# ZhenghaoFei/visual_odom

Hardware: NVIDIA H100
Metric: stereo frames/sec at 1241x376, 2000 feats; LK kernel HBM GB/s vs roofline (higher is better)
Workload: dtype u8/i32 fixed point + f32 (LK), f64 (pose)

## Files before the change

### visual_odom_b200/csrc/batch.cu

```cuda
#include "ctx.h"
#include <string.h>
#include <algorithm>

__global__ void k_pack_counts(vo_unit_result_dev* res, const int* n_pts, const int* n_det, const int* n3, const int* n5,
                              int n_units, int detect)
{
    const int u = blockIdx.x * blockDim.x + threadIdx.x;
    if (u >= n_units) return;
    res[u].n_features = n_pts[u];
    res[u].n_detected = detect ? n_det[u] : 0;
    res[u].n_tracked = n3[u];
    res[u].n_valid = n5[u];
}

#define VO_OUT_BYTES_PER_SLOT (4 * sizeof(float2) + sizeof(int) + sizeof(float3) + sizeof(int))
__global__ void k_pack_outputs(uint8_t* __restrict__ out, size_t stride, int per, const float2* __restrict__ valid4, size_t cs,
                               const int* __restrict__ idx5, const float3* __restrict__ X, const int* __restrict__ inliers,
                               const int* __restrict__ n5, const vo_unit_result_dev* __restrict__ res, int cap)
{
    const int u = blockIdx.x;
    const int nv = min(n5[u], per), ni = min(res[u].n_inliers, per);
    float2* o4 = reinterpret_cast<float2*>(out + (size_t)u * stride);
    int* ok = reinterpret_cast<int*>(o4 + 4 * (size_t)per);
    float* oX = reinterpret_cast<float*>(ok + per);
// ... 159 lines not shown
    char who[64];
    snprintf(who, sizeof(who), "vo_batch_submit_device: unit %d", u);
    const vo_dimage* imgs[4] = {&U.l0, &U.r0, &U.l1, &U.r1};
    static const char* names[4] = {"l0", "r0", "l1", "r1"};
    for (int k = 0; k < 4; k++) {
        const int rc = vo_check_dimage(ctx, who, names[k], imgs[k], ctx->w);
        if (rc) return rc;
    }
    return VO_OK;
}

template <typename Unit>
static int validate_units(vo_ctx* ctx, const Unit* units, int n_units, size_t pitch, bool* detect_out, int* max_pts_out = nullptr)
{
    if (!ctx || !units) return VO_E_INVALID;
    if (n_units <= 0 || n_units > ctx->batch_units) { vo_set_error(ctx, "n_units=%d outside the configured batch (%d)", n_units, ctx->batch_units); return VO_E_INVALID; }
    const bool detect = (units[0].pts == nullptr);
    int max_pts = 0;
    for (int u = 0; u < n_units; u++) {
        const Unit& U = units[u];
        int rc = check_images(ctx, U, u, pitch);
        if (rc) return rc;
        if ((U.pts == nullptr) != detect) { vo_set_error(ctx, "units must all carry features or all request detection"); return VO_E_INVALID; }
        if (U.n_pts < 0 || U.n_pts > ctx->cap) { vo_set_error(ctx, "unit %d: n_pts=%d outside [0,%d]", u, U.n_pts, ctx->cap); return VO_E_CAPACITY; }
        if (U.n_pts > max_pts) max_pts = U.n_pts;
    }
    *detect_out = detect;
    if (max_pts_out) *max_pts_out = max_pts;
    return vo_ensure_pinned(ctx, batch_pinned_bytes(ctx));
}

extern "C" int vo_batch_upload(vo_ctx* ctx, const vo_unit* units, int n_units, size_t pitch)
{
    bool detect;
    int rc = validate_units(ctx, units, n_units, pitch, &detect);
    if (rc) return rc;
    VO_CUDA_CHECK(cudaSetDevice(ctx->device));
    if ((rc = vo_claim_buffers(ctx, "vo_batch_upload", true))) return rc;
    if ((rc = vo_drain_pending(ctx))) return rc;
    VO_CUDA_CHECK(cudaStreamSynchronize(ctx->stream));
    if ((rc = upload_range(ctx, units, 0, n_units, pitch, ctx->stream, detect))) return rc;
    ctx->batch_uploaded = n_units;
    ctx->batch_detect = detect;
    return VO_OK;
}

static int ensure_helpers(vo_ctx* ctx)
{
    if (ctx->lane[0].pre) return VO_OK;
    int lo = 0, hi = 0;
    VO_CUDA_CHECK(cudaDeviceGetStreamPriorityRange(&lo, &hi));
    for (auto& L : ctx->lane) {
        VO_CUDA_CHECK(cudaStreamCreateWithPriority(&L.pre, cudaStreamNonBlocking, hi));
        L.post = L.pre;
        L.lk = L.side;
    }
    return VO_OK;
}

static int run_range_launch(vo_ctx* ctx, const View& v)
{
    int rc;
    View pre = v, lk = v, post = v;
    cudaEvent_t* ev = nullptr;
    for (auto& L : ctx->lane)
        if (L.side && v.s == L.side) {
            if ((rc = ensure_helpers(ctx))) return rc;
            pre.s = L.pre; lk.s = L.lk; post.s = L.post; ev = L.ev;
        }
    auto hand_over = [&](int k, cudaStream_t from, cudaStream_t to) -> int {
        if (from == to) return VO_OK;
        VO_CUDA_CHECK(cudaEventRecord(ev[k], from));
        VO_CUDA_CHECK(cudaStreamWaitEvent(to, ev[k], 0));
        return VO_OK;
    };
    if ((rc = hand_over(0, v.s, pre.s))) return rc;
    if (ctx->batch_detect) {
        if ((rc = vo_run_fast(ctx, pre, 0, false))) return rc;
        if ((rc = vo_run_select(ctx, pre))) return rc;
    }
    if ((rc = vo_run_pyramid(ctx, v.u0 * v.imgs, v.n * v.imgs, pre.s))) return rc;
    if ((rc = hand_over(1, pre.s, lk.s))) return rc;
    const int ip[4] = {0, 1, 3, 2}, in[4] = {1, 3, 2, 0};
    if ((rc = vo_run_lk_ring(ctx, lk, 4, ip, in, false))) return rc;
    if ((rc = hand_over(2, lk.s, post.s))) return rc;
    if ((rc = vo_run_filter(ctx, post, false))) return rc;
    const size_t cs = (size_t)ctx->units * ctx->cap;
    if ((rc = vo_run_triangulate(ctx, post, ctx->d_valid4, ctx->d_valid4 + cs, ctx->d_n5, ctx->d_cal))) return rc;
    if ((rc = vo_run_pnp(ctx, post, ctx->d_valid4 + 2 * cs, ctx->d_n5, ctx->d_cal))) return rc;
    k_pack_counts<<<(v.n + 63) / 64, 64, 0, post.s>>>(ctx->d_results + v.u0, ctx->d_npts + v.u0, ctx->d_ndet + v.u0, ctx->d_n3 + v.u0,
                                                     ctx->d_n5 + v.u0, v.n, ctx->batch_detect ? 1 : 0);
    ctx->launches += 1;
    VO_CUDA_CHECK(cudaGetLastError());
    return hand_over(3, post.s, v.s);
}

static int run_range(vo_ctx* ctx, int u0, int n, cudaStream_t s)
{
    View v{u0, n, s};
    v.max_pts = range_bound(ctx, u0, n);
    bool on_side = false;
    for (const auto& L : ctx->lane) on_side = on_side || (L.side && s == L.side);
    if (on_side) return run_range_launch(ctx, v);
    GraphKey key{};
    key.kind = GraphKey::BATCH_RANGE; key.s = s; key.tma = ctx->lk_use_tma;
    key.u0 = u0; key.n = n; key.max_pts = v.max_pts; key.detect = ctx->batch_detect;
    return vo_run_graph(ctx, key, [&] { return run_range_launch(ctx, v); });
}

extern "C" int vo_batch_run(vo_ctx* ctx)
{
    if (!ctx) return VO_E_INVALID;
    const int units = ctx->batch_uploaded;
    if (units <= 0) { vo_set_error(ctx, "vo_batch_run: nothing uploaded"); return VO_E_INVALID; }
    { int rcc = vo_claim_buffers(ctx, "vo_batch_run"); if (rcc) return rcc; }
    VO_CUDA_CHECK(cudaSetDevice(ctx->device));
    if (units < 2 || ctx->batch_streams < 2) return run_range(ctx, 0, units, ctx->stream);
    int rc = vo_ensure_lanes(ctx);
    if (rc) return rc;
    VO_CUDA_CHECK(cudaEventRecord(ctx->fork_ev, ctx->stream));
    const int half = (units + 1) / 2;
    for (int c = 0; c < 2; c++) {
        const int u0 = c ? half : 0, n = c ? units - half : half;
        cudaStream_t st = ctx->lane[c].side;
        VO_CUDA_CHECK(cudaStreamWaitEvent(st, ctx->fork_ev, 0));
        if ((rc = run_range(ctx, u0, n, st))) return rc;
        VO_CUDA_CHECK(cudaEventRecord(ctx->lane[c].join, st));
        VO_CUDA_CHECK(cudaStreamWaitEvent(ctx->stream, ctx->lane[c].join, 0));
    }
    return VO_OK;
}

extern "C" int vo_batch_download(vo_ctx* ctx, vo_unit_result* results, int n_units)
{
    if (!ctx || !results) return VO_E_INVALID;
    if (n_units <= 0 || n_units > ctx->batch_uploaded) { vo_set_error(ctx, "n_units=%d outside the resident batch (%d)", n_units, ctx->batch_uploaded); return VO_E_INVALID; }
    static_assert(sizeof(vo_unit_result) == sizeof(vo_unit_result_dev), "result record layout");
    VO_CUDA_CHECK(cudaSetDevice(ctx->device));
    VO_CUDA_CHECK(cudaMemcpyAsync(results, ctx->d_results, (size_t)n_units * sizeof(vo_unit_result), cudaMemcpyDeviceToHost, ctx->stream));
    VO_CUDA_CHECK(cudaStreamSynchronize(ctx->stream));
    return VO_OK;
}

extern "C" int vo_frame_batch(vo_ctx* ctx, const vo_unit* units, int n_units, size_t pitch, vo_unit_result* results)
{
    bool detect;
// ... 192 lines not shown
```

### visual_odom_b200/csrc/ctx.cu

```cuda
#include "ctx.h"
#include <string.h>
#include <stdlib.h>

void vo_set_error(vo_ctx* ctx, const char* fmt, ...)
{
    if (!ctx) return;
    va_list ap;
    va_start(ap, fmt);
    vsnprintf(ctx->err, sizeof(ctx->err), fmt, ap);
    va_end(ap);
}

extern "C" void vo_default_params(vo_params* p)
{
    p->fast_threshold = 20;
    p->fast_nonmax = 1;
    p->lk_win = 21;
    p->lk_max_level = 3;
    p->lk_max_iters = 30;
    p->lk_epsilon = 0.01;
    p->lk_min_eig = 0.001;
    p->circ_threshold = 0;
    p->pnp_iterations = 500;
    p->pnp_reproj_error = 0.5f;
    p->pnp_confidence = (double)0.999f;
    p->max_features = 8192;
    p->max_units = 1;
}

extern "C" int vo_create(int device, const vo_params* params, vo_ctx** out)
{
    if (!out) return VO_E_INVALID;
    *out = nullptr;
    vo_ctx* ctx = new vo_ctx();
    if (params) ctx->p = *params; else vo_default_params(&ctx->p);
    ctx->device = device;
    *out = ctx;
    if (ctx->p.fast_threshold < 0 || ctx->p.fast_threshold > 255) {
        vo_set_error(ctx, "fast_threshold=%d outside [0,255]", ctx->p.fast_threshold);
        return VO_E_INVALID;
    }
    if (ctx->p.lk_win != VO_WIN) {
        vo_set_error(ctx, "lk_win=%d unsupported: the LK kernel is built for the reference's 21x21 window", ctx->p.lk_win);
        return VO_E_UNSUPPORTED;
    }
    if (ctx->p.lk_max_level < 0 || ctx->p.lk_max_level >= VO_MAX_LEVELS) {
        vo_set_error(ctx, "lk_max_level=%d outside [0,%d]", ctx->p.lk_max_level, VO_MAX_LEVELS - 1);
        return VO_E_UNSUPPORTED;
    }
    int ndev = 0;
    cudaError_t e = cudaGetDeviceCount(&ndev);
    if (e != cudaSuccess || ndev <= 0) {
        vo_set_error(ctx, "no CUDA device available (%s): this library has no CPU fallback", cudaGetErrorString(e));
        return VO_E_CUDA;
    }
    VO_CUDA_CHECK(cudaSetDevice(device));
    cudaDeviceProp prop;
    VO_CUDA_CHECK(cudaGetDeviceProperties(&prop, device));
    if (prop.major != 9 || prop.minor != 0) {
        vo_set_error(ctx, "device %d is sm_%d%d; this library ships sm_90a code only", device, prop.major, prop.minor);
        return VO_E_UNSUPPORTED;
    }
    ctx->sm_count = prop.multiProcessorCount;
    VO_CUDA_CHECK(cudaStreamCreateWithFlags(&ctx->own_stream, cudaStreamNonBlocking));
    ctx->stream = ctx->own_stream;
    VO_CUDA_CHECK(vo_lk_prepare());
    ctx->cap = ctx->p.max_features;
    VO_CUDA_CHECK(cudaMalloc(&ctx->d_lk_queue, LK_QUEUES * 2 * sizeof(int)));
    VO_CUDA_CHECK(cudaMemset(ctx->d_lk_queue, 0, LK_QUEUES * 2 * sizeof(int)));
    {
        const char* st = getenv("VO_LK_STAGING");
        ctx->lk_use_tma = !(st && strcmp(st, "ldg") == 0);
        const char* sp = getenv("VO_LK_SPAN");
        if (sp) ctx->lk_span = atoi(sp);
    }
    return VO_OK;
}

extern "C" void vo_destroy(vo_ctx* ctx)
{
    if (!ctx) return;
    cudaSetDevice(ctx->device);
    vo_drain_pending(ctx);
    if (ctx->stream) cudaStreamSynchronize(ctx->stream);
    vo_dist_shutdown(ctx);
    vo_partition_destroy(ctx);
    vo_free_state(ctx);
    for (cudaEvent_t e : ctx->ev_pool) cudaEventDestroy(e);
    for (auto& p : ctx->pending) if (p.done) cudaEventDestroy(p.done);
    for (int k = 0; k < 2; k++) {
        if (ctx->seq_front_ev[k]) cudaEventDestroy(ctx->seq_front_ev[k]);
        if (ctx->seq_back_ev[k]) cudaEventDestroy(ctx->seq_back_ev[k]);
    }
    if (ctx->fork_ev) cudaEventDestroy(ctx->fork_ev);
    for (auto& L : ctx->lane) {
        if (L.join) cudaEventDestroy(L.join);
        if (L.side) cudaStreamDestroy(L.side);
        for (cudaEvent_t e : L.ev) if (e) cudaEventDestroy(e);
    }
    if (ctx->h_pinned) cudaFreeHost(ctx->h_pinned);
    if (ctx->d_bgr) cudaFree(ctx->d_bgr);
    if (ctx->d_lk_queue) cudaFree(ctx->d_lk_queue);
    if (ctx->d_ess) cudaFree(ctx->d_ess);
    if (ctx->d_seq_ess) cudaFree(ctx->d_seq_ess);
    for (int k = 0; k < 2; k++) if (ctx->seq_mono_ev[k]) cudaEventDestroy(ctx->seq_mono_ev[k]);
    if (ctx->seq_mono_stream) cudaStreamDestroy(ctx->seq_mono_stream);
    if (ctx->h_out) cudaFreeHost(ctx->h_out);
    if (ctx->own_stream) cudaStreamDestroy(ctx->own_stream);
    delete ctx;
}

extern "C" const char* vo_last_error(const vo_ctx* ctx) { return ctx ? ctx->err : "null context"; }

extern "C" int vo_set_stream(vo_ctx* ctx, void* s)
{
    if (!ctx) return VO_E_INVALID;
    VO_CUDA_CHECK(cudaStreamSynchronize(ctx->stream));
    ctx->stream = s ? (cudaStream_t)s : ctx->own_stream;
    return VO_OK;
}

extern "C" int vo_sync(vo_ctx* ctx)
{
    if (!ctx) return VO_E_INVALID;
    VO_CUDA_CHECK(cudaStreamSynchronize(ctx->stream));
    return VO_OK;
}

extern "C" int vo_set_option(vo_ctx* ctx, const char* key, double value)
{
    if (!ctx || !key) return VO_E_INVALID;
    if (strcmp(key, "batch_streams") == 0) { ctx->batch_streams = value >= 2 ? 2 : 1; return VO_OK; }
    if (strcmp(key, "lk_staging") == 0) { ctx->lk_use_tma = !(value >= 1); return VO_OK; }
    if (strcmp(key, "batch_outputs") == 0) { ctx->batch_outputs = value >= 1; vo_drop_graphs(ctx); return VO_OK; }
    if (strcmp(key, "sm_partition") == 0) {
        if (value < 0) { vo_set_error(ctx, "sm_partition=%g: the number of SMs must not be negative", value); return VO_E_INVALID; }
        ctx->part_auto = false;
        return vo_partition_enable(ctx, (int)value);
    }
    if (strcmp(key, "lk_span") == 0) { ctx->lk_span = (int)value; vo_drop_graphs(ctx); return VO_OK; }
    if (strcmp(key, "graphs") == 0) { ctx->use_graphs = value >= 1; return VO_OK; }
    if (strcmp(key, "mono_rotation") == 0) { ctx->mono_opt = value >= 1; vo_drop_graphs(ctx); return VO_OK; }
    vo_set_error(ctx, "unknown option %s", key);
    return VO_E_INVALID;
}

extern "C" long long vo_kernel_launches(const vo_ctx* ctx) { return ctx ? ctx->launches : 0; }

extern "C" int vo_lk_kernel_time(vo_ctx* ctx, double* ms_total, long long* n, int reset)
{
    if (!ctx) return VO_E_INVALID;
    VO_CUDA_CHECK(cudaStreamSynchronize(ctx->stream));
    for (size_t i = 0; i + 1 < ctx->ev_used; i += 2) {
        float ms = 0.f;
        VO_CUDA_CHECK(cudaEventElapsedTime(&ms, ctx->ev_pool[i], ctx->ev_pool[i + 1]));
        ctx->lk_ms += ms;
        ctx->lk_n++;
    }
    ctx->ev_used = 0;
    if (ms_total) *ms_total = ctx->lk_ms;
    if (n) *n = ctx->lk_n;
    if (reset) { ctx->lk_ms = 0.0; ctx->lk_n = 0; }
    return VO_OK;
}

int vo_ensure_pinned(vo_ctx* ctx, size_t bytes)
{
    if (bytes <= ctx->h_pinned_bytes) return VO_OK;
    if (ctx->h_pinned) { cudaFreeHost(ctx->h_pinned); ctx->h_pinned = nullptr; ctx->h_pinned_bytes = 0; }
    VO_CUDA_CHECK(cudaMallocHost(&ctx->h_pinned, bytes));
    ctx->h_pinned_bytes = bytes;
    return VO_OK;
}

int vo_upload_plane(vo_ctx* ctx, uint8_t* dst, const uint8_t* src, size_t row_bytes, int h, size_t pitch, cudaStream_t st)
{
    if (pitch == row_bytes) VO_CUDA_CHECK(cudaMemcpyAsync(dst, src, row_bytes * h, cudaMemcpyHostToDevice, st));
    else VO_CUDA_CHECK(cudaMemcpy2DAsync(dst, row_bytes, src, pitch, row_bytes, h, cudaMemcpyHostToDevice, st));
    return VO_OK;
}

int vo_refuse_pending_batches(vo_ctx* ctx, const char* who)
{
    for (auto& p : ctx->pending)
        if (p.active) {
            vo_set_error(ctx, "%s: the vo_batch_submit submission of slots [%d, %d) has not been waited for", who, p.u0, p.u0 + p.n);
            return VO_E_INVALID;
        }
    return VO_OK;
}

int vo_claim_buffers(vo_ctx* ctx, const char* who, bool allow_pending_batches)
{
    if (ctx->seq_inflight > 0) {
        vo_set_error(ctx, "%s: %d frame(s) submitted with vo_seq_submit have not been waited for (this call would overwrite their buffers)", who, ctx->seq_inflight);
        return VO_E_INVALID;
    }
    int rc;
    if (!allow_pending_batches && (rc = vo_refuse_pending_batches(ctx, who))) return rc;
    ctx->seq_active = false;
    return VO_OK;
}

typedef CUresult (*PFN_cuDeviceGet)(CUdevice*, int);
typedef CUresult (*PFN_cuDeviceGetDevResource)(CUdevice, CUdevResource*, CUdevResourceType);
typedef CUresult (*PFN_cuDevSmResourceSplitByCount)(CUdevResource*, unsigned int*, const CUdevResource*, CUdevResource*, unsigned int, unsigned int);
typedef CUresult (*PFN_cuDevResourceGenerateDesc)(CUdevResourceDesc*, CUdevResource*, unsigned int);
typedef CUresult (*PFN_cuGreenCtxCreate)(CUgreenCtx*, CUdevResourceDesc, CUdevice, unsigned int);
typedef CUresult (*PFN_cuGreenCtxStreamCreate)(CUstream*, CUgreenCtx, unsigned int, int);
typedef CUresult (*PFN_cuGreenCtxDestroy)(CUgreenCtx);

template <typename F>
static bool drv(const char* name, F* fn)
{
    void* p = nullptr;
    cudaDriverEntryPointQueryResult q;
    if (cudaGetDriverEntryPoint(name, &p, cudaEnableDefault, &q) != cudaSuccess || q != cudaDriverEntryPointSuccess || !p) return false;
    *fn = (F)p;
    return true;
}

void vo_partition_destroy(vo_ctx* ctx)
{
    for (auto& L : ctx->lane) {
        if (L.pre) cudaStreamDestroy(L.pre);
        if (L.post && L.post != L.pre) cudaStreamDestroy(L.post);
        L.pre = L.lk = L.post = nullptr;
    }
    PFN_cuGreenCtxDestroy destroy = nullptr;
    if (drv("cuGreenCtxDestroy", &destroy))
        for (int k = 0; k < 2; k++) if (ctx->part_gctx[k]) destroy((CUgreenCtx)ctx->part_gctx[k]);
    ctx->part_gctx[0] = ctx->part_gctx[1] = nullptr;
    ctx->part_on = false; ctx->part_helper_sms = ctx->part_lk_sms = 0;
}

int vo_partition_enable(vo_ctx* ctx, int helper_sms)
{
    VO_CUDA_CHECK(cudaSetDevice(ctx->device));
    int rc = vo_drain_pending(ctx);
    if (rc) return rc;
    VO_CUDA_CHECK(cudaDeviceSynchronize());
    vo_drop_graphs(ctx);
    vo_partition_destroy(ctx);
    if (helper_sms <= 0) return VO_OK;
    PFN_cuDeviceGet dget; PFN_cuDeviceGetDevResource getres; PFN_cuDevSmResourceSplitByCount split;
    PFN_cuDevResourceGenerateDesc gendesc; PFN_cuGreenCtxCreate create; PFN_cuGreenCtxStreamCreate screate;
    if (!drv("cuDeviceGet", &dget) || !drv("cuDeviceGetDevResource", &getres) || !drv("cuDevSmResourceSplitByCount", &split) ||
        !drv("cuDevResourceGenerateDesc", &gendesc) || !drv("cuGreenCtxCreate", &create) || !drv("cuGreenCtxStreamCreate", &screate)) {
        vo_set_error(ctx, "sm_partition: this driver has no green-context API");
        return VO_E_UNSUPPORTED;
    }
    CUdevice dev;
    CUdevResource all, part[1], rest;
    unsigned int nb = 1;
    CUresult r;
    if ((r = dget(&dev, ctx->device)) != CUDA_SUCCESS || (r = getres(dev, &all, CU_DEV_RESOURCE_TYPE_SM)) != CUDA_SUCCESS ||
        (r = split(part, &nb, &all, &rest, 0, (unsigned)helper_sms)) != CUDA_SUCCESS || nb != 1) {
        vo_set_error(ctx, "sm_partition: splitting off %d SMs failed (driver error %d)", helper_sms, (int)r);
        return VO_E_UNSUPPORTED;
    }
    CUdevResource* rs[2] = {&part[0], &rest};
    for (int k = 0; k < 2; k++) {
        CUdevResourceDesc desc;
        CUgreenCtx g;
        if ((r = gendesc(&desc, rs[k], 1)) != CUDA_SUCCESS || (r = create(&g, desc, dev, CU_GREEN_CTX_DEFAULT_STREAM)) != CUDA_SUCCESS) {
            vo_set_error(ctx, "sm_partition: cuGreenCtxCreate failed (driver error %d)", (int)r);
            vo_partition_destroy(ctx);
            return VO_E_UNSUPPORTED;
        }
        ctx->part_gctx[k] = g;
    }
    ctx->part_helper_sms = (int)part[0].sm.smCount; ctx->part_lk_sms = (int)rest.sm.smCount;
    for (int c = 0; c < VO_LANES; c++) {
        CUstream a, b;
        if ((r = screate(&a, (CUgreenCtx)ctx->part_gctx[0], CU_STREAM_NON_BLOCKING, 0)) != CUDA_SUCCESS ||
            (r = screate(&b, (CUgreenCtx)ctx->part_gctx[1], CU_STREAM_NON_BLOCKING, 0)) != CUDA_SUCCESS) {
            vo_set_error(ctx, "sm_partition: cuGreenCtxStreamCreate failed (driver error %d)", (int)r);
            vo_partition_destroy(ctx);
            return VO_E_UNSUPPORTED;
        }
        vo_ctx::Lane& L = ctx->lane[c];
        L.pre = L.lk = (cudaStream_t)b;
        L.post = (cudaStream_t)a;
    }
    ctx->part_on = true;
    return VO_OK;
}

int vo_drain_pending(vo_ctx* ctx)
{
    for (auto& p : ctx->pending)
        if (p.active) {
            VO_CUDA_CHECK(cudaEventSynchronize(p.done));
            p.active = false;
        }
    if (ctx->seq_inflight > 0 && ctx->lane[0].side) VO_CUDA_CHECK(cudaStreamSynchronize(ctx->lane[0].side));
    return VO_OK;
}

void vo_drop_graphs(vo_ctx* ctx)
{
    for (auto& g : ctx->graphs) cudaGraphExecDestroy(g.exec);
    ctx->graphs.clear();
}

static bool same_key(const GraphKey& a, const GraphKey& b)
{
    return a.kind == b.kind && a.s == b.s && a.tma == b.tma && a.u0 == b.u0 && a.n == b.n && a.max_pts == b.max_pts &&
           a.detect == b.detect && a.slot == b.slot && a.parity == b.parity && a.bgr == b.bgr;
}

int vo_run_graph(vo_ctx* ctx, const GraphKey& key, const std::function<int()>& launch)
{
    if (!ctx->use_graphs) return launch();
    for (auto& g : ctx->graphs)
        if (same_key(g.key, key)) {
            VO_CUDA_CHECK(cudaGraphLaunch(g.exec, key.s));
            ctx->launches += g.launches;
            return VO_OK;
        }
    const bool timing = ctx->lk_timing;
    const long long before = ctx->launches;
    ctx->lk_timing = false;
    cudaGraph_t graph = nullptr;
    VO_CUDA_CHECK(cudaStreamBeginCapture(key.s, cudaStreamCaptureModeThreadLocal));
    int rc = launch();
    cudaError_t e = cudaStreamEndCapture(key.s, &graph);
    ctx->lk_timing = timing;
    if (rc) { if (graph) cudaGraphDestroy(graph); return rc; }
    VO_CUDA_CHECK(e);
    vo_ctx::CachedGraph g;
    g.key = key;
    g.launches = ctx->launches - before;
    VO_CUDA_CHECK(cudaGraphInstantiate(&g.exec, graph, 0));
    cudaGraphDestroy(graph);
    ctx->graphs.push_back(g);
    VO_CUDA_CHECK(cudaGraphLaunch(g.exec, key.s));
    return VO_OK;
}

int vo_ensure_lanes(vo_ctx* ctx)
{
    if (ctx->fork_ev) return VO_OK;
    VO_CUDA_CHECK(cudaEventCreateWithFlags(&ctx->fork_ev, cudaEventDisableTiming));
    for (auto& L : ctx->lane) {
        VO_CUDA_CHECK(cudaStreamCreateWithFlags(&L.side, cudaStreamNonBlocking));
        VO_CUDA_CHECK(cudaEventCreateWithFlags(&L.join, cudaEventDisableTiming));
        for (cudaEvent_t& e : L.ev) VO_CUDA_CHECK(cudaEventCreateWithFlags(&e, cudaEventDisableTiming));
    }
    return VO_OK;
}

int vo_write_calib(vo_ctx* ctx, int u0, int n, const CamCalib* c)
{
    const size_t e0 = (size_t)(1 + u0);
    if (memcmp(ctx->cal.data() + e0, c, n * sizeof(CamCalib)) == 0) return VO_OK;
    memcpy(ctx->cal.data() + e0, c, n * sizeof(CamCalib));
    for (auto& p : ctx->pending)
        if (p.active) VO_CUDA_CHECK(cudaStreamWaitEvent(ctx->stream, p.done, 0));
    VO_CUDA_CHECK(cudaMemcpyAsync(ctx->d_cal_tab + e0, ctx->cal.data() + e0, n * sizeof(CamCalib), cudaMemcpyHostToDevice, ctx->stream));
    return VO_OK;
}

int vo_set_calibration(vo_ctx* ctx, int u0, int n, const float* P_l, const float* P_r, int n_mat)
{
    std::vector<CamCalib> c(n);
    for (int i = 0; i < n; i++) c[i] = vo_calib_from(P_l + 12 * (i % n_mat), P_r + 12 * (i % n_mat));
    return vo_write_calib(ctx, u0, n, c.data());
}

void vo_free_state(vo_ctx* ctx)
{
    vo_drop_graphs(ctx);
    for (void* p : ctx->allocs) cudaFree(p);
    ctx->allocs.clear();
    if (ctx->d_seq_state) cudaFree(ctx->d_seq_state);
    ctx->d_seq_state = nullptr; ctx->seq_n_cap = 0;
    ctx->d_feat_pts = nullptr; ctx->d_feat_ages = nullptr; ctx->d_feat_cnt = ctx->d_bucket = ctx->d_seq_err = ctx->d_seq_live = nullptr;
    ctx->d_out = nullptr; ctx->out_stride = 0; ctx->out_per = 0;
    ctx->d_cal_tab = ctx->d_cal = nullptr;
    ctx->w = ctx->h = ctx->units = 0;
}

template <typename T>
static cudaError_t dalloc(vo_ctx* ctx, T** p, size_t count)
{
    void* q = nullptr;
    cudaError_t e = cudaMalloc(&q, count * sizeof(T) + 256);
    if (e == cudaSuccess) { ctx->allocs.push_back(q); *p = (T*)q; }
    return e;
}

typedef CUresult (*PFN_encodeTiled)(CUtensorMap*, CUtensorMapDataType, cuuint32_t, void*, const cuuint64_t*,
                                    const cuuint64_t*, const cuuint32_t*, const cuuint32_t*, CUtensorMapInterleave,
                                    CUtensorMapSwizzle, CUtensorMapL2promotion, CUtensorMapFloatOOBfill);

static int encode_maps(vo_ctx* ctx)
{
    void* fn = nullptr;
    cudaDriverEntryPointQueryResult qres;
    VO_CUDA_CHECK(cudaGetDriverEntryPoint("cuTensorMapEncodeTiled", &fn, cudaEnableDefault, &qres));
// ... 151 lines not shown
{
    const size_t uo = (size_t)v.u0 * ctx->cap;
    const PyrGeom& pg = ctx->pg;

    LkArgs a;
    memset(&a, 0, sizeof(a));
    a.n_units = v.n;
    a.cap = ctx->cap;
    a.n_pts = ctx->d_npts + v.u0;
    a.imgs_per_unit = v.imgs;
    a.img_plane0 = v.plane0 >= 0 ? v.plane0 : v.u0 * v.imgs;
    a.ncalls = ncalls;
    for (int c = 0; c < ncalls; c++) { a.img_prev[c] = img_prev[c]; a.img_next[c] = img_next[c]; }
    a.nlevels = pg.nlevels;
    for (int l = 0; l < pg.nlevels; l++) { a.lw[l] = pg.lv[l].w; a.lh[l] = pg.lv[l].h; }
    a.max_iters = ctx->p.lk_max_iters;
    double eps = ctx->p.lk_epsilon;
    if (eps < 0.) eps = 0.; if (eps > 10.) eps = 10.;
    a.eps2 = eps * eps;
    a.min_eig = ctx->p.lk_min_eig;
    a.pts_in = ctx->d_pts_in + uo;
    a.pts_out = ctx->d_pts_out + uo;
    a.status_out = ctx->d_status + uo;
    a.err_out = want_err ? ctx->d_err + uo : nullptr;
    a.call_stride = (size_t)ctx->units * ctx->cap;
    a.use_tma = ctx->lk_use_tma ? 1 : 0;
    for (int l = 0; l < pg.nlevels; l++) {
        a.img_base[l] = ctx->pg.lv[l].img; a.der_base[l] = ctx->pg.lv[l].der;
        a.pitch[l] = pg.lv[l].pitch; a.plane[l] = pg.lv[l].plane;
    }

    cudaEvent_t e0 = nullptr, e1 = nullptr;
    if (ctx->lk_timing) {
        if (ctx->ev_used + 2 > ctx->ev_pool.size()) {
            cudaEvent_t a0, a1;
            VO_CUDA_CHECK(cudaEventCreate(&a0));
            VO_CUDA_CHECK(cudaEventCreate(&a1));
            ctx->ev_pool.push_back(a0); ctx->ev_pool.push_back(a1);
        }
        e0 = ctx->ev_pool[ctx->ev_used]; e1 = ctx->ev_pool[ctx->ev_used + 1];
        ctx->ev_used += 2;
        VO_CUDA_CHECK(cudaEventRecord(e0, v.s));
    }
    {
        size_t qi = 0;
        while (qi < ctx->lk_queue_streams.size() && ctx->lk_queue_streams[qi] != v.s) qi++;
        if (qi == ctx->lk_queue_streams.size()) {
            if (qi >= LK_QUEUES) { vo_set_error(ctx, "more than %d streams launch the LK kernel", LK_QUEUES); return VO_E_CAPACITY; }
            ctx->lk_queue_streams.push_back(v.s);
        }
        a.queue = ctx->d_lk_queue + 2 * qi;
        a.per_unit = v.max_pts > 0 && v.max_pts < ctx->cap ? v.max_pts : ctx->cap;
        a.progress = ctx->d_lk_progress + uo;
        int lk_sms = ctx->sm_count;
        for (const auto& L : ctx->lane) if (ctx->part_on && v.s == L.lk) lk_sms = ctx->part_lk_sms;
        const bool big = (long)a.n_units * a.per_unit > (long)lk_sms * LK_CTAS_PER_SM * LK_WARPS_PER_CTA;
        a.span = ctx->lk_span > 0 ? ctx->lk_span : (big ? 2 : 0);
        VO_CUDA_CHECK(vo_launch_lk_ring(ctx->maps, a, lk_sms, v.s));
    }
    ctx->launches += 1;
    if (e1) VO_CUDA_CHECK(cudaEventRecord(e1, v.s));
    return VO_OK;
}

int vo_run_filter(vo_ctx* ctx, const View& v, bool with_ages)
{
    const size_t uo = (size_t)v.u0 * ctx->cap;
    FilterArgs f;
    memset(&f, 0, sizeof(f));
    f.cap = ctx->cap;
    f.call_stride = (size_t)ctx->units * ctx->cap;
    f.circ_threshold = ctx->p.circ_threshold;
    f.n_pts = ctx->d_npts + v.u0;
    f.pts_in = ctx->d_pts_in + uo;
    f.pts_out = ctx->d_pts_out + uo;
    f.status = ctx->d_status + uo;
    f.ages_in = with_ages ? ctx->d_ages_in + uo : nullptr;
    f.ages_out = ctx->d_ages_out + uo;
    f.kept5 = ctx->d_kept5 + uo;
    f.idx3 = ctx->d_idx3 + uo;
    f.n3 = ctx->d_n3 + v.u0;
    f.valid4 = ctx->d_valid4 + uo;
    f.idx5 = ctx->d_idx5 + uo;
    f.n5 = ctx->d_n5 + v.u0;
    VO_CUDA_CHECK(vo_launch_ring_filter(f, v.n, v.s));
    ctx->launches += 1;
    return VO_OK;
}

int vo_run_fast(vo_ctx* ctx, const View& v, int plane_in_unit, bool want_resp)
{
    FastArgs a;
    memset(&a, 0, sizeof(a));
    const size_t plane = (size_t)ctx->w * ctx->h;
    a.n_units = v.n;
    a.img_tab = ctx->d_raw_tab + (size_t)(v.plane0 >= 0 ? v.plane0 : v.u0 * v.imgs) + plane_in_unit;
    a.img_stride_idx = v.imgs;
    a.w = ctx->w; a.h = ctx->h; a.pitch = ctx->w;
    a.threshold = ctx->p.fast_threshold; a.nonmax = ctx->p.fast_nonmax;
    a.score = ctx->d_score + v.u0 * plane; a.score_plane = plane;
    a.rowbuf = ctx->d_rowbuf + v.u0 * plane; a.rowcap = ctx->w;
    a.rowcount = ctx->d_rowcount + (size_t)v.u0 * ctx->h; a.rowoff = ctx->d_rowoff + (size_t)v.u0 * ctx->h;
    a.n_det = ctx->d_ndet + v.u0;
    a.corners = ctx->d_corners + (size_t)v.u0 * ctx->corner_cap;
    a.resp = want_resp ? ctx->d_resp + (size_t)v.u0 * ctx->corner_cap : nullptr;
    a.corner_cap = ctx->corner_cap;
    ctx->launches += vo_launch_fast(a, v.s);
    VO_CUDA_CHECK(cudaGetLastError());
    return VO_OK;
}

// ... 42 lines not shown
```

### visual_odom_b200/csrc/ctx.h

```cpp
#pragma once
#include "common.cuh"
#include "lk_ring.h"
#include "filter.h"
#include "fast.h"
#include "pnp.h"
#include "seq.h"
#include "ess.h"
#include "../../include/vo_b200.h"
#include <vector>
#include <functional>
#include <stdarg.h>
#define LK_QUEUES 32
#define VO_DIST_BUCKET 4
#define VO_DIST_NB 4
#define VO_LANES 3

struct GraphKey {
    enum Kind { BATCH_RANGE, SEQ_FRONT, SEQ_BACK } kind;
    cudaStream_t s;
    bool tma;
    int u0, n, max_pts; bool detect;
    int slot, parity; bool bgr;
};

// ... 69 lines not shown
    uint8_t* d_bgr = nullptr;
    size_t bgr_bytes = 0;
    bool part_on = false;
    bool part_auto = true;
    int part_helper_sms = 0, part_lk_sms = 0;
    void* part_gctx[2] = {nullptr, nullptr};
    void* dist_comm = nullptr;
    int dist_rank = 0, dist_world = 1;
    cudaStream_t dist_stream = nullptr, dist_snap_stream = nullptr;
    struct DistBucket { void* d = nullptr; void* h = nullptr; cudaEvent_t done = nullptr; int fill = 0, unwaited = 0, n_units = 0; bool flushed = false; };
    struct DistStep { int bucket = 0, index = 0; };
    DistBucket dist_bk[VO_DIST_NB];
    DistStep dist_steps[2 * VO_DIST_DEPTH];
    int dist_cur = 0;
    cudaEvent_t dist_ev_read = nullptr, dist_ev_fork = nullptr;
    size_t dist_bytes = 0;
    long long dist_head = 0, dist_tail = 0;
    void* d_ess = nullptr;
    int ess_cap = 0;
    bool mono_opt = false;
    bool seq_mono = false;
    void* d_seq_ess = nullptr;
    size_t seq_ess_bytes = 0;
    int seq_ess_cap = 0;
    int seq_ess_units = 0;
    cudaStream_t seq_mono_stream = nullptr;
    cudaEvent_t seq_mono_ev[2] = {nullptr, nullptr};
    std::vector<void*> allocs;

    void* h_pinned = nullptr;
    size_t h_pinned_bytes = 0;

    std::vector<cudaEvent_t> ev_pool;
    size_t ev_used = 0;
    double lk_ms = 0.0;
    long long lk_n = 0;
    bool lk_timing = true;
    bool lk_use_tma = true;
    int lk_span = 0;
    int* d_lk_progress = nullptr;
    int* d_lk_queue = nullptr;
    std::vector<cudaStream_t> lk_queue_streams;

    int batch_units = 0;
    int batch_uploaded = 0;
    bool batch_detect = false;
    int batch_streams = 2;
    bool use_graphs = true;
    struct CachedGraph { GraphKey key; cudaGraphExec_t exec; long long launches; };
    std::vector<CachedGraph> graphs;
    std::vector<int> slot_pts;
    struct Lane {
        cudaStream_t side = nullptr;
        cudaStream_t pre = nullptr, lk = nullptr, post = nullptr;
        cudaEvent_t join = nullptr, ev[4] = {};
    };
    Lane lane[VO_LANES];
    cudaEvent_t fork_ev = nullptr;
    struct Pending { int u0 = 0, n = 0; bool active = false; cudaEvent_t done = nullptr; };
    std::vector<Pending> pending;
    bool batch_outputs = false;
    uint8_t* d_out = nullptr;
    uint8_t* h_out = nullptr;
    size_t out_stride = 0;
    int out_per = 0, out_units = 0;
    unsigned submit_count = 0;
};

void vo_set_error(vo_ctx* ctx, const char* fmt, ...);
int vo_ensure_state(vo_ctx* ctx, int w, int h, int units);
void vo_free_state(vo_ctx* ctx);
void vo_drop_graphs(vo_ctx* ctx);
int vo_run_graph(vo_ctx* ctx, const GraphKey& key, const std::function<int()>& launch);
int vo_ensure_lanes(vo_ctx* ctx);
int vo_write_calib(vo_ctx* ctx, int u0, int n, const CamCalib* c);
int vo_set_calibration(vo_ctx* ctx, int u0, int n, const float* P_l, const float* P_r, int n_mat);
int vo_drain_pending(vo_ctx* ctx);
int vo_partition_enable(vo_ctx* ctx, int helper_sms);
void vo_partition_destroy(vo_ctx* ctx);
int vo_dist_order_after_gathers(vo_ctx* ctx, cudaStream_t st);
void vo_dist_shutdown(vo_ctx* ctx);
int vo_claim_buffers(vo_ctx* ctx, const char* who, bool allow_pending_batches = false);
int vo_refuse_pending_batches(vo_ctx* ctx, const char* who);
int vo_ensure_pinned(vo_ctx* ctx, size_t bytes);
int vo_upload_plane(vo_ctx* ctx, uint8_t* dst, const uint8_t* src, size_t row_bytes, int h, size_t pitch, cudaStream_t st);
int vo_ensure_bgr(vo_ctx* ctx, size_t bytes);
int vo_launch_bgr_to_gray(const vo_dimage* d_tab, const vo_dimage& packed, size_t packed_stride, uint8_t* d_gray, size_t img_stride_out,
                          int w, int h, int n_img, cudaStream_t s);
vo_dimage vo_packed_bgr(const uint8_t* d_bgr, int w);
int vo_check_dimage(vo_ctx* ctx, const char* who, const char* name, const vo_dimage* im, int w);
int vo_ingest_device(vo_ctx* ctx, const vo_dimage* h_tab, int n, int plane0, cudaStream_t st);
struct View { int u0, n; cudaStream_t s; int plane0 = -1; int imgs = 4; int max_pts = 0; };
int vo_run_lk(vo_ctx* ctx, const View& v, int ncalls, const int* img_prev, const int* img_next, bool want_err);
int vo_run_pyramid(vo_ctx* ctx, int plane0, int nplanes, cudaStream_t s);
int vo_run_lk_ring(vo_ctx* ctx, const View& v, int ncalls, const int* img_prev, const int* img_next, bool want_err);
int vo_run_filter(vo_ctx* ctx, const View& v, bool with_ages);
int vo_run_fast(vo_ctx* ctx, const View& v, int plane_in_unit, bool want_resp);
int vo_run_select(vo_ctx* ctx, const View& v);
int vo_run_triangulate(vo_ctx* ctx, const View& v, const float2* pts_l, const float2* pts_r, const int* n, const CamCalib* cal,
                       float4* X4 = nullptr);
int vo_run_pnp(vo_ctx* ctx, const View& v, const float2* pts2d, const int* n, const CamCalib* cal);
```

### visual_odom_b200/csrc/lk_ring.cu

```cuda
#include "common.cuh"
#include "lk_ring.h"

#define FULL 0xffffffffu
#define W_BITS 14

namespace {

template <bool B> struct BoolC { static constexpr bool value = B; };

__device__ __forceinline__ uint32_t smem_u32(const void* p)
{
    return (uint32_t)__cvta_generic_to_shared(p);
}
__device__ __forceinline__ void mbar_init(uint64_t* bar, uint32_t count)
{
    asm volatile("mbarrier.init.shared::cta.b64 [%0], %1;" ::"r"(smem_u32(bar)), "r"(count) : "memory");
}
__device__ __forceinline__ void mbar_expect_tx(uint64_t* bar, uint32_t bytes)
{
    asm volatile("mbarrier.arrive.expect_tx.shared::cta.b64 _, [%0], %1;" ::"r"(smem_u32(bar)), "r"(bytes)
                 : "memory");
}
__device__ __forceinline__ void mbar_wait(uint64_t* bar, uint32_t parity)
{
// ... 447 lines not shown
                                }
                                mbar_wait(&sm.bar, phase); phase ^= 1;
                            } else {
                                ldg_box_u8(sm.jtile, args.img_base[0] + args.plane[0] * img_next, args.pitch[0], jbx, jby, J_ROWS, lane);
                                __syncwarp();
                            }
                        }
                        a = fxp - (float)inx; b = fyp - (float)iny;
                        bilinear_weights(a, b, w00, w01, w10, w11);
                        const unsigned wt = (unsigned)w00 | ((unsigned)w01 << 16), wb = (unsigned)w10 | ((unsigned)(w11 & 0xffff) << 16);
                        int s = 0;
#pragma unroll
                        for (int part = 0; part < 2; part++) {
                            const int c0 = part ? tcol : col, row0 = part ? tr0 : r0, ne = part ? 4 : 11, nvalid = part ? tn : nvalid_s;
                            const int joff = (ry + row0) * TW + rx + c0;
                            const uint32_t* jw = reinterpret_cast<const uint32_t*>(sm.jtile) + (joff >> 2);
                            const int jsh = 8 * (joff & 3);
                            unsigned ptop = __funnelshift_r(jw[0], jw[1], jsh);
#pragma unroll
                            for (int k = 0; k < ne; k++) {
                                const unsigned pbot = __funnelshift_r(jw[(k + 1) * TWW], jw[(k + 1) * TWW + 1], jsh);
                                const int e = part ? 11 + k : k;
                                const int Iv = (e & 1) ? (Ipk[e >> 1] >> 16) : (int)(short)(Ipk[e >> 1] & 0xffff);
                                const int diff = (dp2a_taps(wb, pbot, dp2a_taps(wt, ptop, 1 << (W_BITS - 6))) >> (W_BITS - 5)) - Iv;
                                if (k < nvalid) s += abs(diff);
                                ptop = pbot;
                            }
                        }
                        s = __reduce_add_sync(FULL, s);
                        errv = __fdiv_rn(__fmul_rn((float)s, 1.f), (float)(32 * VO_WIN * VO_WIN));
                    }
                }
            } while (0);

            if (level == 0) {
                if (lane == 0) {
                    const size_t o = (size_t)call * args.call_stride + pbase;
                    args.pts_out[o] = nxt;
                    args.status_out[o] = (uint8_t)status;
                    if (args.err_out) args.err_out[o] = errv;
                }
                pt = nxt;
                status = 1; errv = 0.f;
            }
        }
        if (span < nphases && lane == 0) {
            const int last_level = max_level - ((p1 - 1) - call * args.nlevels);
            if (last_level != 0) args.pts_out[(size_t)call * args.call_stride + pbase] = nxt;
            st_release(args.progress + pbase, p1 == nphases ? 0 : p1);
        }
    }

    if (lane == 0) {
        const int total_warps = gridDim.x * LK_WARPS_PER_CTA;
        if (atomicAdd(args.queue + 1, 1) == total_warps - 1) {
            args.queue[1] = 0;
            __threadfence();
            args.queue[0] = 0;
        }
    }
}

size_t vo_lk_smem_bytes() { return sizeof(WarpSmem) * LK_WARPS_PER_CTA; }

template <bool T>
static cudaError_t prep()
{
    return cudaFuncSetAttribute(k_lk_ring<T>, cudaFuncAttributeMaxDynamicSharedMemorySize, (int)vo_lk_smem_bytes());
}

cudaError_t vo_lk_prepare()
{
    cudaError_t e = prep<false>();
    return e != cudaSuccess ? e : prep<true>();
}

cudaError_t vo_launch_lk_ring(const LkMaps& maps, const LkArgs& args, int sm_count, cudaStream_t stream)
{
    const long items = (long)args.n_units * args.per_unit;
    if (items <= 0) return cudaSuccess;
    const long resident = (long)(sm_count > 0 ? sm_count : 148) * LK_CTAS_PER_SM;
    long ctas = (items + LK_WARPS_PER_CTA - 1) / LK_WARPS_PER_CTA;
    if (ctas > resident) ctas = resident;
    const int thr = LK_WARPS_PER_CTA * 32;
    const size_t sh = vo_lk_smem_bytes();
    if (args.use_tma) k_lk_ring<true><<<(int)ctas, thr, sh, stream>>>(maps, args);
    else k_lk_ring<false><<<(int)ctas, thr, sh, stream>>>(maps, args);
    return cudaGetLastError();
}
```

### visual_odom_b200/csrc/lk_ring.h

```cpp
#pragma once
#include "common.cuh"

#define LK_WARPS_PER_CTA 2
#define LK_CTAS_PER_SM 8

struct LkMaps {
    CUtensorMap img_i[VO_MAX_LEVELS];
    CUtensorMap img_j[VO_MAX_LEVELS];
    CUtensorMap der[VO_MAX_LEVELS];
};

struct LkArgs {
    int n_units;
    int cap;
    const int* n_pts;
    int imgs_per_unit;
    int img_plane0;
    int ncalls;
    int img_prev[4];
    int img_next[4];
    int nlevels;
    int lw[VO_MAX_LEVELS], lh[VO_MAX_LEVELS];
    int max_iters;
    double eps2;
    double min_eig;
    const float2* pts_in;
    float2* pts_out;
    uint8_t* status_out;
    float* err_out;
    size_t call_stride;
    int* queue;
    int per_unit;
    int span;
    int* progress;
    int use_tma;
    const uint8_t* img_base[VO_MAX_LEVELS];
    const uint32_t* der_base[VO_MAX_LEVELS];
    int pitch[VO_MAX_LEVELS];
    size_t plane[VO_MAX_LEVELS];
};

size_t vo_lk_smem_bytes();
cudaError_t vo_lk_prepare();
cudaError_t vo_launch_lk_ring(const LkMaps& maps, const LkArgs& args, int sm_count, cudaStream_t stream);
int vo_launch_pyramid(const PyrGeom& pg, const uint8_t* const* src_tab_dev, int src_pitch, cudaStream_t stream);
```

Before: 4147.

## Overlap pyramid build with FAST detection and optionally share LK across partitions

When detection runs on a side lane, the image pyramid is now built on its own high-priority stream so it can run at the same time as FAST and selection. LK waits on both. An optional lk_share mode (off by default) launches a second LK ring grid on the helper green-context partition. The two grids share the work queue through an explicit participant count, so idle helper SMs can take LK items. This adds cross-stream event dependencies, including a tail event to order reuse, and risks contention between concurrent kernels.

```diff
diff --git a/visual_odom_b200/csrc/batch.cu b/visual_odom_b200/csrc/batch.cu
--- a/visual_odom_b200/csrc/batch.cu
+++ b/visual_odom_b200/csrc/batch.cu
@@ -235,6 +235,7 @@
     VO_CUDA_CHECK(cudaDeviceGetStreamPriorityRange(&lo, &hi));
     for (auto& L : ctx->lane) {
         VO_CUDA_CHECK(cudaStreamCreateWithPriority(&L.pre, cudaStreamNonBlocking, hi));
+        VO_CUDA_CHECK(cudaStreamCreateWithPriority(&L.pyr, cudaStreamNonBlocking, hi));
         L.post = L.pre;
         L.lk = L.side;
     }
@@ -246,10 +247,11 @@
     int rc;
     View pre = v, lk = v, post = v;
     cudaEvent_t* ev = nullptr;
+    vo_ctx::Lane* lane = nullptr;
     for (auto& L : ctx->lane)
         if (L.side && v.s == L.side) {
             if ((rc = ensure_helpers(ctx))) return rc;
-            pre.s = L.pre; lk.s = L.lk; post.s = L.post; ev = L.ev;
+            pre.s = L.pre; lk.s = L.lk; post.s = L.post; ev = L.ev; lane = &L;
         }
     auto hand_over = [&](int k, cudaStream_t from, cudaStream_t to) -> int {
         if (from == to) return VO_OK;
@@ -258,11 +260,17 @@
         return VO_OK;
     };
     if ((rc = hand_over(0, v.s, pre.s))) return rc;
+    const bool split = lane && ctx->batch_detect;
+    if (split) VO_CUDA_CHECK(cudaStreamWaitEvent(lane->pyr, ev[0], 0));
     if (ctx->batch_detect) {
         if ((rc = vo_run_fast(ctx, pre, 0, false))) return rc;
         if ((rc = vo_run_select(ctx, pre))) return rc;
     }
-    if ((rc = vo_run_pyramid(ctx, v.u0 * v.imgs, v.n * v.imgs, pre.s))) return rc;
+    if ((rc = vo_run_pyramid(ctx, v.u0 * v.imgs, v.n * v.imgs, split ? lane->pyr : pre.s))) return rc;
+    if (split) {
+        VO_CUDA_CHECK(cudaEventRecord(lane->pyr_ev, lane->pyr));
+        VO_CUDA_CHECK(cudaStreamWaitEvent(lk.s, lane->pyr_ev, 0));
+    }
     if ((rc = hand_over(1, pre.s, lk.s))) return rc;
     const int ip[4] = {0, 1, 3, 2}, in[4] = {1, 3, 2, 0};
     if ((rc = vo_run_lk_ring(ctx, lk, 4, ip, in, false))) return rc;
@@ -275,6 +283,7 @@
                                                      ctx->d_n5 + v.u0, v.n, ctx->batch_detect ? 1 : 0);
     ctx->launches += 1;
     VO_CUDA_CHECK(cudaGetLastError());
+    if (ev) VO_CUDA_CHECK(cudaEventRecord(ctx->tail_ev, post.s));
     return hand_over(3, post.s, v.s);
 }
 
diff --git a/visual_odom_b200/csrc/ctx.cu b/visual_odom_b200/csrc/ctx.cu
--- a/visual_odom_b200/csrc/ctx.cu
+++ b/visual_odom_b200/csrc/ctx.cu
@@ -73,6 +73,8 @@
         ctx->lk_use_tma = !(st && strcmp(st, "ldg") == 0);
         const char* sp = getenv("VO_LK_SPAN");
         if (sp) ctx->lk_span = atoi(sp);
+        const char* sh = getenv("VO_LK_SHARE");
+        if (sh) ctx->lk_share = atoi(sh) != 0;
     }
     return VO_OK;
 }
@@ -93,10 +95,13 @@
         if (ctx->seq_back_ev[k]) cudaEventDestroy(ctx->seq_back_ev[k]);
     }
     if (ctx->fork_ev) cudaEventDestroy(ctx->fork_ev);
+    if (ctx->tail_ev) cudaEventDestroy(ctx->tail_ev);
     for (auto& L : ctx->lane) {
         if (L.join) cudaEventDestroy(L.join);
         if (L.side) cudaStreamDestroy(L.side);
         for (cudaEvent_t e : L.ev) if (e) cudaEventDestroy(e);
+        for (cudaEvent_t e : L.share_ev) if (e) cudaEventDestroy(e);
+        if (L.pyr_ev) cudaEventDestroy(L.pyr_ev);
     }
     if (ctx->h_pinned) cudaFreeHost(ctx->h_pinned);
     if (ctx->d_bgr) cudaFree(ctx->d_bgr);
@@ -139,6 +144,7 @@
         return vo_partition_enable(ctx, (int)value);
     }
     if (strcmp(key, "lk_span") == 0) { ctx->lk_span = (int)value; vo_drop_graphs(ctx); return VO_OK; }
+    if (strcmp(key, "lk_share") == 0) { ctx->lk_share = value >= 1; return VO_OK; }
     if (strcmp(key, "graphs") == 0) { ctx->use_graphs = value >= 1; return VO_OK; }
     if (strcmp(key, "mono_rotation") == 0) { ctx->mono_opt = value >= 1; vo_drop_graphs(ctx); return VO_OK; }
     vo_set_error(ctx, "unknown option %s", key);
@@ -225,7 +231,8 @@
     for (auto& L : ctx->lane) {
         if (L.pre) cudaStreamDestroy(L.pre);
         if (L.post && L.post != L.pre) cudaStreamDestroy(L.post);
-        L.pre = L.lk = L.post = nullptr;
+        if (L.pyr) cudaStreamDestroy(L.pyr);
+        L.pre = L.lk = L.post = L.pyr = nullptr;
     }
     PFN_cuGreenCtxDestroy destroy = nullptr;
     if (drv("cuGreenCtxDestroy", &destroy))
@@ -272,16 +279,18 @@
     }
     ctx->part_helper_sms = (int)part[0].sm.smCount; ctx->part_lk_sms = (int)rest.sm.smCount;
     for (int c = 0; c < VO_LANES; c++) {
-        CUstream a, b;
-        if ((r = screate(&a, (CUgreenCtx)ctx->part_gctx[0], CU_STREAM_NON_BLOCKING, 0)) != CUDA_SUCCESS ||
-            (r = screate(&b, (CUgreenCtx)ctx->part_gctx[1], CU_STREAM_NON_BLOCKING, 0)) != CUDA_SUCCESS) {
+        CUstream a = nullptr, b = nullptr, p = nullptr;
+        vo_ctx::Lane& L = ctx->lane[c];
+        if ((r = screate(&a, (CUgreenCtx)ctx->part_gctx[0], CU_STREAM_NON_BLOCKING, 0)) == CUDA_SUCCESS) L.post = (cudaStream_t)a;
+        if (r == CUDA_SUCCESS && (r = screate(&b, (CUgreenCtx)ctx->part_gctx[1], CU_STREAM_NON_BLOCKING, 0)) == CUDA_SUCCESS)
+            L.pre = L.lk = (cudaStream_t)b;
+        if (r == CUDA_SUCCESS && (r = screate(&p, (CUgreenCtx)ctx->part_gctx[1], CU_STREAM_NON_BLOCKING, 0)) == CUDA_SUCCESS)
+            L.pyr = (cudaStream_t)p;
+        if (r != CUDA_SUCCESS) {
             vo_set_error(ctx, "sm_partition: cuGreenCtxStreamCreate failed (driver error %d)", (int)r);
             vo_partition_destroy(ctx);
             return VO_E_UNSUPPORTED;
         }
-        vo_ctx::Lane& L = ctx->lane[c];
-        L.pre = L.lk = (cudaStream_t)b;
-        L.post = (cudaStream_t)a;
     }
     ctx->part_on = true;
     return VO_OK;
@@ -343,10 +352,13 @@
 {
     if (ctx->fork_ev) return VO_OK;
     VO_CUDA_CHECK(cudaEventCreateWithFlags(&ctx->fork_ev, cudaEventDisableTiming));
+    VO_CUDA_CHECK(cudaEventCreateWithFlags(&ctx->tail_ev, cudaEventDisableTiming));
     for (auto& L : ctx->lane) {
         VO_CUDA_CHECK(cudaStreamCreateWithFlags(&L.side, cudaStreamNonBlocking));
         VO_CUDA_CHECK(cudaEventCreateWithFlags(&L.join, cudaEventDisableTiming));
         for (cudaEvent_t& e : L.ev) VO_CUDA_CHECK(cudaEventCreateWithFlags(&e, cudaEventDisableTiming));
+        for (cudaEvent_t& e : L.share_ev) VO_CUDA_CHECK(cudaEventCreateWithFlags(&e, cudaEventDisableTiming));
+        VO_CUDA_CHECK(cudaEventCreateWithFlags(&L.pyr_ev, cudaEventDisableTiming));
     }
     return VO_OK;
 }
@@ -604,11 +616,26 @@
         a.queue = ctx->d_lk_queue + 2 * qi;
         a.per_unit = v.max_pts > 0 && v.max_pts < ctx->cap ? v.max_pts : ctx->cap;
         a.progress = ctx->d_lk_progress + uo;
-        int lk_sms = ctx->sm_count;
-        for (const auto& L : ctx->lane) if (ctx->part_on && v.s == L.lk) lk_sms = ctx->part_lk_sms;
+        vo_ctx::Lane* lane = nullptr;
+        for (auto& L : ctx->lane) if (ctx->part_on && v.s == L.lk) lane = &L;
+        const int lk_sms = lane ? ctx->part_lk_sms : ctx->sm_count;
         const bool big = (long)a.n_units * a.per_unit > (long)lk_sms * LK_CTAS_PER_SM * LK_WARPS_PER_CTA;
         a.span = ctx->lk_span > 0 ? ctx->lk_span : (big ? 2 : 0);
-        VO_CUDA_CHECK(vo_launch_lk_ring(ctx->maps, a, lk_sms, v.s));
+        const bool share = lane && ctx->lk_share && a.span > 0 && a.span < ncalls * pg.nlevels;
+        const int ctas = vo_lk_ctas(a, lk_sms), helper_ctas = share ? vo_lk_ctas(a, ctx->part_helper_sms) : 0;
+        a.participants = (ctas + helper_ctas) * LK_WARPS_PER_CTA;
+        if (lane) VO_CUDA_CHECK(cudaStreamWaitEvent(v.s, lane->share_ev[1], 0));
+        if (helper_ctas > 0) {
+            VO_CUDA_CHECK(cudaEventRecord(lane->share_ev[0], v.s));
+            VO_CUDA_CHECK(cudaStreamWaitEvent(lane->post, lane->share_ev[0], 0));
+            VO_CUDA_CHECK(cudaStreamWaitEvent(lane->post, ctx->tail_ev, 0));
+        }
+        VO_CUDA_CHECK(vo_launch_lk_ring(ctx->maps, a, ctas, v.s));
+        if (helper_ctas > 0) {
+            VO_CUDA_CHECK(vo_launch_lk_ring(ctx->maps, a, helper_ctas, lane->post));
+            VO_CUDA_CHECK(cudaEventRecord(lane->share_ev[1], lane->post));
+            ctx->launches += 1;
+        }
     }
     ctx->launches += 1;
     if (e1) VO_CUDA_CHECK(cudaEventRecord(e1, v.s));
diff --git a/visual_odom_b200/csrc/ctx.h b/visual_odom_b200/csrc/ctx.h
--- a/visual_odom_b200/csrc/ctx.h
+++ b/visual_odom_b200/csrc/ctx.h
@@ -145,11 +145,15 @@
     std::vector<int> slot_pts;
     struct Lane {
         cudaStream_t side = nullptr;
-        cudaStream_t pre = nullptr, lk = nullptr, post = nullptr;
+        cudaStream_t pre = nullptr, lk = nullptr, post = nullptr, pyr = nullptr;
         cudaEvent_t join = nullptr, ev[4] = {};
+        cudaEvent_t share_ev[2] = {};
+        cudaEvent_t pyr_ev = nullptr;
     };
     Lane lane[VO_LANES];
     cudaEvent_t fork_ev = nullptr;
+    cudaEvent_t tail_ev = nullptr;
+    bool lk_share = false;
     struct Pending { int u0 = 0, n = 0; bool active = false; cudaEvent_t done = nullptr; };
     std::vector<Pending> pending;
     bool batch_outputs = false;
diff --git a/visual_odom_b200/csrc/lk_ring.cu b/visual_odom_b200/csrc/lk_ring.cu
--- a/visual_odom_b200/csrc/lk_ring.cu
+++ b/visual_odom_b200/csrc/lk_ring.cu
@@ -523,8 +523,7 @@
     }
 
     if (lane == 0) {
-        const int total_warps = gridDim.x * LK_WARPS_PER_CTA;
-        if (atomicAdd(args.queue + 1, 1) == total_warps - 1) {
+        if (atomicAdd(args.queue + 1, 1) == args.participants - 1) {
             args.queue[1] = 0;
             __threadfence();
             args.queue[0] = 0;
@@ -546,16 +545,22 @@
     return e != cudaSuccess ? e : prep<true>();
 }
 
-cudaError_t vo_launch_lk_ring(const LkMaps& maps, const LkArgs& args, int sm_count, cudaStream_t stream)
+int vo_lk_ctas(const LkArgs& args, int sm_count)
 {
     const long items = (long)args.n_units * args.per_unit;
-    if (items <= 0) return cudaSuccess;
+    if (items <= 0) return 0;
     const long resident = (long)(sm_count > 0 ? sm_count : 148) * LK_CTAS_PER_SM;
     long ctas = (items + LK_WARPS_PER_CTA - 1) / LK_WARPS_PER_CTA;
     if (ctas > resident) ctas = resident;
+    return (int)ctas;
+}
+
+cudaError_t vo_launch_lk_ring(const LkMaps& maps, const LkArgs& args, int ctas, cudaStream_t stream)
+{
+    if (ctas <= 0) return cudaSuccess;
     const int thr = LK_WARPS_PER_CTA * 32;
     const size_t sh = vo_lk_smem_bytes();
-    if (args.use_tma) k_lk_ring<true><<<(int)ctas, thr, sh, stream>>>(maps, args);
-    else k_lk_ring<false><<<(int)ctas, thr, sh, stream>>>(maps, args);
+    if (args.use_tma) k_lk_ring<true><<<ctas, thr, sh, stream>>>(maps, args);
+    else k_lk_ring<false><<<ctas, thr, sh, stream>>>(maps, args);
     return cudaGetLastError();
 }
diff --git a/visual_odom_b200/csrc/lk_ring.h b/visual_odom_b200/csrc/lk_ring.h
--- a/visual_odom_b200/csrc/lk_ring.h
+++ b/visual_odom_b200/csrc/lk_ring.h
@@ -30,6 +30,7 @@
     float* err_out;
     size_t call_stride;
     int* queue;
+    int participants;
     int per_unit;
     int span;
     int* progress;
@@ -42,5 +43,6 @@
 
 size_t vo_lk_smem_bytes();
 cudaError_t vo_lk_prepare();
-cudaError_t vo_launch_lk_ring(const LkMaps& maps, const LkArgs& args, int sm_count, cudaStream_t stream);
+int vo_lk_ctas(const LkArgs& args, int sm_count);
+cudaError_t vo_launch_lk_ring(const LkMaps& maps, const LkArgs& args, int ctas, cudaStream_t stream);
 int vo_launch_pyramid(const PyrGeom& pg, const uint8_t* const* src_tab_dev, int src_pitch, cudaStream_t stream);
```

Result: no change. 4186, median of 6 (+0.9%).
